# tmuird/VAEUNET

Measured on AMD Instinct MI355X. Metric: images/sec (whole node) at 3x512x512 bs=8/GPU; Dice parity vs CPU ref, higher is better.
Workload: dtype bf16; 1 GPU; UNet(3,2) train step (fwd+CombinedLoss+bwd+clip+AdamW), random-init weights; image=3x512x512, batch_per_gpu=8, global_batch=8, parallelism=dp1, execution=hipgraph-replay, wgrad_side_stream=False

## Files before the change

include/vaeunet.h:

```cpp
#ifndef VAEUNET_H
#define VAEUNET_H
#include <stdint.h>
#ifdef __cplusplus
extern "C" {
#endif

typedef struct VuGather {
  const void* src[3];
  int64_t stride[3];
  int32_t cend[3];
  int32_t nsrc;
  int32_t C;
  int32_t N, H, W;
  int32_t Hs, Ws;
  int32_t R, S;
  int32_t sy, sx, dy, dx, oy, ox;
} VuGather;

typedef struct VuGemmFwd {
  VuGather a;
  const void* b;
  int64_t ldb;
  int32_t ncol;
  int32_t out_mode;
// ... 216 lines not shown
                    int dtype, void* stream);
int vu_attn_gate_fwd(const float* q, const float* st, const void* x,
                     int64_t xs, int64_t P, int C, float* pmap, void* out,
                     int64_t os, int dtype, void* stream);
int vu_attn_gate_bwd(const void* dout, int64_t dos, const void* x, int64_t xs,
                     const float* pmap, int64_t P, int C, void* dx,
                     int64_t dxs, float* dqpre, int dtype, void* stream);
int64_t vu_attn_psi_bwd_workspace_bytes(int64_t P, int F);
int vu_attn_psi_bwd(const void* ug, const void* ux, int64_t P, int F,
                    const float* sg, const float* tg, const float* sx,
                    const float* tx, const float* wpsi, const float* dq,
                    void* ds, float* dwpsi, float* dbpsi, int accumulate,
                    float* workspace, int dtype, void* stream);
int64_t vu_attn_psi_bwd_blocks(int64_t P);
int vu_attn_psi_bwd_bnb_ok(int F);
int vu_attn_psi_bwd_bnb(const void* ug, const void* ux, int64_t P, int F,
                        const float* sg, const float* tg, const float* sx,
                        const float* tx, const float* wpsi, const float* dq,
                        void* ds, float* dwpsi, float* dbpsi, int accumulate,
                        float* workspace, const float* mean_g, const float* invstd_g,
                        const float* mean_x, const float* invstd_x, float* bnb_g,
                        float* bnb_x, int dtype, void* stream);

int64_t vu_attn_tail_bwd_tile(int F, int C);
int vu_attn_tail_bwd_ok(int64_t P, int F, int C, int64_t ldg, int64_t ldx, int64_t dos,
                        int64_t dgs, int64_t dg_coff, int64_t dxs, int dtype);
int vu_attn_tail_bwd(const void* ug, const void* ux, const float* dq, int64_t P, int F, int C,
                     const float* sg, const float* tg, const float* sx, const float* tx,
                     const float* wpsi, const float* mean_g, const float* coef_g,
                     const float* mean_x, const float* coef_x, const void* wdg, int64_t ldg,
                     const void* wdx, int64_t ldx, const void* dout, int64_t dos,
                     const float* pmap, void* dg, int64_t dgs, int64_t dg_coff, int dg_acc,
                     void* dx, int64_t dxs, void* dug, void* dux, int dtype, void* stream);

int vu_pointwise_fwd(const void* x, int64_t xs, int64_t P, int C, int J,
                     const float* w, const float* b, float* y, int64_t ys,
                     int dtype, void* stream);
int64_t vu_pointwise_bwd_workspace_bytes(int64_t P, int C, int J);
int vu_pointwise_bwd(const void* x, int64_t xs, const float* dy, int64_t dys,
                     int64_t P, int C, int J, const float* w, void* dx,
                     int64_t dxs, float* dw, float* db, int accumulate,
                     float* workspace, int dtype, void* stream);
int vu_pointwise_bn_fwd(const void* x, int64_t xs, int64_t P, int C, int J,
                        const float* bn_scale, const float* bn_shift, const float* w,
                        const float* b, float* y, int64_t ys, int dtype, void* stream);
int64_t vu_pointwise_bn_bwd_blocks(int64_t P);
int vu_pointwise_bn_bwd(const void* x, int64_t xs, const float* bn_coef, int64_t coef_stride,
                        const float* dy, int64_t dys, int64_t P, int C, int J, const float* w,
                        void* dx, int64_t dxs, float* dw, float* db, int accumulate,
                        float* workspace, float* bnb, int dtype, void* stream);

int64_t vu_loss_workspace_bytes(void);
int vu_bce_dice_fwd2(const float* logits, const float* target, int64_t n,
                     double* sums, float smooth, float w_bce, float w_dice,
                     float* loss, float* parts, double* workspace,
                     void* stream);
int vu_bce_dice_fwd(const float* logits, const float* target, int64_t n,
                    double* sums, double* workspace, void* stream);
int vu_bce_dice_bwd(const float* logits, const float* target, int64_t n,
                    const double* sums, float smooth, float w_bce,
                    float w_dice, const float* gscale, float* grad,
                    void* stream);
int vu_kl_free_bits2(const float* mu, const float* logvar, int B, int L,
                     float free_bits, const float* gscale, float* value,
                     float* gmu, float* glogvar, void* stream);
int vu_kl_free_bits(const float* mu, const float* logvar, int B, int L,
// ... 188 lines not shown
```

vaeunet_amd/_lib.py:

```python
import ctypes as C
import os

import torch

_HERE = os.path.dirname(os.path.abspath(__file__))
LIB_PATH = os.path.join(_HERE, "libvaeunet_hip.so")
if os.environ.get("VU_LIB_PATH"):
    LIB_PATH = os.environ["VU_LIB_PATH"]

F32, BF16 = 0, 1

_p = C.c_void_p
_i = C.c_int
_l = C.c_int64
_f = C.c_float


class VuGather(C.Structure):
    _fields_ = [("src", _p * 3), ("stride", _l * 3), ("cend", C.c_int32 * 3),
                ("nsrc", C.c_int32), ("C", C.c_int32),
                ("N", C.c_int32), ("H", C.c_int32), ("W", C.c_int32),
                ("Hs", C.c_int32), ("Ws", C.c_int32), ("R", C.c_int32), ("S", C.c_int32),
                ("sy", C.c_int32), ("sx", C.c_int32), ("dy", C.c_int32), ("dx", C.c_int32),
                ("oy", C.c_int32), ("ox", C.c_int32)]
# ... 102 lines not shown
    "vu_bn_bwd_reduce": (_i, [_p, _l, _p, _l, _l, _i, _p, _p, _p, _p, _p, _i, _i, _p, _p, _i,
                              _p, _p, _i, _p]),
    "vu_bn_bwd_apply": (_i, [_p, _l, _p, _l, _l, _i, _p, _p, _p, _p, _i, _p, _l, _i, _p]),
    "vu_bn_bwd_apply2_ok": (_i, [_i, _l, _l, _l, _l, _l]),
    "vu_bn_bwd_apply2": (_i, [_p, _l, _p, _l, _p, _l, _l, _i, _p, _p, _p, _p, _p, _l, _p, _l, _i, _p]),
    "vu_reduce_workspace_bytes": (_l, [_l, _i]),
    "vu_chan_sum": (_i, [_p, _l, _i, _i, _i, _i, _i, _i, _i, _i, _p, _i, _p, _i, _p]),
    "vu_copy": (_i, [_p, _l, _i, _p, _l, _i, _l, _i, _i, _p]),
    "vu_zero": (_i, [_p, _l, _l, _i, _i, _p]),
    "vu_gpu_delay": (_i, [_i, _p]),
    "vu_zero_insert2": (_i, [_p, _l, _i, _i, _i, _i, _p, _l, _i, _i, _i, _p]),
    "vu_input_pack": (_i, [_p, _l, _l, _l, _l, _i, _i, _i, _i, _i, _p, _i, _p]),
    "vu_maxpool2_fwd": (_i, [_p, _l, _i, _i, _i, _i, _p, _l, _i, _p]),
    "vu_maxpool2_bwd": (_i, [_p, _l, _p, _l, _i, _i, _i, _i, _p, _l, _p, _l, _i, _p]),
    "vu_bn_apply_maxpool2": (_i, [_p, _l, _p, _l, _p, _l, _i, _i, _i, _i, _p, _p, _i, _i, _p]),
    "vu_upsample_fwd": (_i, [_p, _l, _i, _i, _i, _i, _p, _l, _i, _i, _i, _i, _i, _i, _i, _p]),
    "vu_upsample_bwd": (_i, [_p, _l, _i, _i, _i, _i, _p, _l, _i, _i, _i, _i, _i, _i, _i, _i,
                             _p]),
    "vu_attn_tile_rows": (_l, []),
    "vu_attn_psi_fwd": (_i, [_p, _p, _l, _i, _p, _p, _p, _p, _p, _p, _p, _p, _p, _l, _i, _p]),
    "vu_attn_gate_fwd": (_i, [_p, _p, _p, _l, _l, _i, _p, _p, _l, _i, _p]),
    "vu_attn_gate_bwd": (_i, [_p, _l, _p, _l, _p, _l, _i, _p, _l, _p, _i, _p]),
    "vu_attn_psi_bwd_workspace_bytes": (_l, [_l, _i]),
    "vu_attn_psi_bwd_blocks": (_l, [_l]),
    "vu_attn_psi_bwd_bnb_ok": (_i, [_i]),
    "vu_attn_psi_bwd_bnb": (_i, [_p, _p, _l, _i, _p, _p, _p, _p, _p, _p, _p, _p, _p, _i, _p, _p, _p, _p, _p, _p, _p,
                                 _i, _p]),
    "vu_attn_psi_bwd": (_i, [_p, _p, _l, _i, _p, _p, _p, _p, _p, _p, _p, _p, _p, _i, _p, _i,
                             _p]),
    "vu_attn_tail_bwd_tile": (_l, [_i, _i]),
    "vu_attn_tail_bwd_ok": (_i, [_l, _i, _i, _l, _l, _l, _l, _l, _l, _i]),
    "vu_attn_tail_bwd": (_i, [_p, _p, _p, _l, _i, _i, _p, _p, _p, _p, _p, _p, _p, _p, _p, _p, _l, _p, _l, _p, _l,
                              _p, _p, _l, _l, _i, _p, _l, _p, _p, _i, _p]),
    "vu_pointwise_fwd": (_i, [_p, _l, _l, _i, _i, _p, _p, _p, _l, _i, _p]),
    "vu_pointwise_bwd_workspace_bytes": (_l, [_l, _i, _i]),
    "vu_pointwise_bn_fwd": (_i, [_p, _l, _l, _i, _i, _p, _p, _p, _p, _p, _l, _i, _p]),
    "vu_pointwise_bn_bwd_blocks": (_l, [_l]),
    "vu_pointwise_bn_bwd": (_i, [_p, _l, _p, _l, _p, _l, _l, _i, _i, _p, _p, _l, _p, _p, _i, _p, _p, _i, _p]),
    "vu_pointwise_bwd": (_i, [_p, _l, _p, _l, _l, _i, _i, _p, _p, _l, _p, _p, _i, _p, _i, _p]),
    "vu_loss_workspace_bytes": (_l, []),
    "vu_bce_dice_fwd2": (_i, [_p, _p, _l, _p, _f, _f, _f, _p, _p, _p, _p]),
    "vu_bce_dice_bwd": (_i, [_p, _p, _l, _p, _f, _f, _f, _p, _p, _p]),
    "vu_kl_free_bits2": (_i, [_p, _p, _i, _i, _f, _p, _p, _p, _p, _p]),
    "vu_sumsq": (_i, [_p, _l, _p, _p, _p]),
    "vu_dice_score": (_i, [_p, _p, _l, _f, _p, _p, _p, _p]),
    "vu_seg_counts_workspace_bytes": (_l, [_l]),
    "vu_seg_counts": (_i, [_p, _i, C.POINTER(_l), _i, _i, _p, _i, C.POINTER(_l), _i, _i, _i, _i, _i, _i, _p, _i, _p,
                           _p, _p]),
    "vu_seg_metrics": (_i, [_p, _i, _i, C.c_double, _p, _p, _i, _p, _p]),
    "vu_mt_chunk_elems": (_l, []),
    "vu_mt_grad_norm": (_i, [_p, _i, _l, _f, _p, _p, _p, _p]),
    "vu_mt_scale_grads": (_i, [_p, _i, _l, _p, _p]),
    "vu_mt_adamw": (_i, [_p, _i, _l, _f, _f, _f, _f, _f, _p, _p]),
    "vu_mt_adamw_dev": (_i, [_p, _i, _l, C.c_double, C.c_double, C.c_double, C.c_double, C.c_double, _p, _i,
                             _p]),
    "vu_mt_adamw_dev_scaled": (_i, [_p, _i, _l, C.c_double, C.c_double, C.c_double, C.c_double, C.c_double, _p,
                                    _i, _p, _p]),
    "vu_maxpool3s2_fwd": (_i, [_p, _l, _i, _i, _i, _i, _p, _l, _p, _i, _p]),
    "vu_maxpool3s2_bwd": (_i, [_p, _l, _p, _i, _i, _i, _i, _p, _l, _i, _i, _p]),
    "vu_bn_add_relu": (_i, [_p, _l, _p, _p, _p, _l, _p, _p, _l, _i, _p, _l, _i, _p]),
    "vu_relu_mask": (_i, [_p, _l, _p, _l, _l, _i, _p, _l, _i, _p]),
    "vu_sample_sum": (_i, [_p, _l, _i, _i, _i, _f, _p, _i, _p, _i, _p]),
    "vu_sample_sum_workspace_bytes": (_l, [_i, _i]),
    "vu_sample_broadcast": (_i, [_p, _i, _i, _i, _f, _p, _l, _i, _i, _p]),
    "vu_linear_small_fwd": (_i, [_p, _i, _i, _p, _p, _i, _p, _p]),
    "vu_linear_small_bwd": (_i, [_p, _i, _i, _p, _i, _p, _p, _i, _p, _p, _i, _p]),
# ... 67 lines not shown
```

vaeunet_amd/csrc/attention_tail.hip:

```cpp
#include <type_traits>

#include "host.h"
#include "attn_pre.h"

namespace {

VU_DEV uint32_t pack2(float a, float b) { return (uint32_t)f2bf(a) | ((uint32_t)f2bf(b) << 16); }

enum { Q_SG, Q_TG, Q_SX, Q_TX, Q_WP, Q_MG, Q_AG, Q_BG, Q_EG, Q_MX, Q_AX, Q_BX, Q_EX, NQ };

struct AttnTail {
  const bf16_t *ug, *ux;
  const float *dq, *pmap;
  const float* coef[NQ];
  const bf16_t *wg, *wx;
  int64_t ldg, ldx;
  const bf16_t* dout;
  int64_t dos;
  bf16_t* dg;
  int64_t dgs;
  int dg_acc;
  bf16_t* dx;
  int64_t dxs;
  bf16_t *dug, *dux;
  int64_t P;
};

template <int KS, int NJ, int NF, int NW>
__global__ __launch_bounds__(64 * NW, NW == 4 ? 2 : 1) void attn_tail_kernel(AttnTail p) {
  constexpr int K = 32 * KS, N = 16 * NJ, PX = 16 * NF, NT = 64 * NW;
  constexpr int GS = 4;
  static_assert(NJ % GS == 0, "whole 64-column groups");
  __shared__ __attribute__((aligned(16))) char wsm[2][N * K * 2];
  __shared__ __attribute__((aligned(16))) float csm[NQ][K];

  const int ntiles = (int)(p.P / PX);
  const int lane = threadIdx.x & 63;
  const int wid = __builtin_amdgcn_readfirstlane(threadIdx.x >> 6);
  const int gq = lane >> 4, r16 = lane & 15;

  auto wrow = [&](int j, int r) { return (j / GS) * 16 * GS + 4 * GS * (r >> 2) + 4 * (j % GS) + (r & 3); };
  {
    constexpr int PIECES = NJ * KS * 64;
#pragma unroll
    for (int img = 0; img < 2; ++img) {
      const bf16_t* bmat = img ? p.wx : p.wg;
      const int64_t ld = img ? p.ldx : p.ldg;
      for (int e = threadIdx.x; e < PIECES; e += NT) {
        const int l = e & 63, jk = e >> 6, j = jk / KS, ks = jk - j * KS;
        *reinterpret_cast<u32x4*>(wsm[img] + e * 16) =
            *reinterpret_cast<const u32x4*>(bmat + (int64_t)wrow(j, l & 15) * ld + 32 * ks + 8 * (l >> 4));
      }
    }
#pragma unroll
    for (int q = 0; q < NQ; ++q)
      for (int c = threadIdx.x; c < K; c += NT) csm[q][c] = p.coef[q][c];
    __syncthreads();
  }

  const int tstride = gridDim.x * NW;
  auto tile_px = [&](int t) {
    asm volatile("" : "+s"(t));
    return (int64_t)t * PX;
  };
  auto opq = [](uint32_t v) {
    asm volatile("" : "+v"(v));
    return v;
  };
  const uint32_t lk0 = (uint32_t)(r16 * K + 8 * gq);
  auto load = [&](int t, u32x4 (&a)[NF][KS], u32x4 (&b)[NF][KS], float (&g)[NF], float (&pv)[NF]) {
    const int64_t pb = tile_px(t);
    const uint32_t lk = opq(lk0), lr = opq((uint32_t)r16);
    const bf16_t *ugb = p.ug + pb * K + lk, *uxb = p.ux + pb * K + lk;
    const float *dqb = p.dq + pb + lr, *pmb = p.pmap + pb + lr;
#pragma unroll
    for (int f = 0; f < NF; ++f) {
      g[f] = dqb[16 * f];
      pv[f] = pmb[16 * f];
#pragma unroll
      for (int ks = 0; ks < KS; ++ks) {
        a[f][ks] = *reinterpret_cast<const u32x4*>(ugb + 16 * f * K + 32 * ks);
        b[f][ks] = *reinterpret_cast<const u32x4*>(uxb + 16 * f * K + 32 * ks);
      }
    }
  };
  u32x4 na[NF][KS], nb[NF][KS];
  float ng[NF], npv[NF];
  int tile = blockIdx.x * NW + wid;
  if (tile < ntiles) load(tile, na, nb, ng, npv);
  for (; tile < ntiles; tile += tstride) {
    const int64_t pb = tile_px(tile);
    int lo = 0;
    asm volatile("" : "+v"(lo));
    auto coef8 = [&](int q, int ks, float (&d)[8]) {
      const char* s = reinterpret_cast<const char*>(&csm[q][32 * ks + 8 * gq]) + lo;
      const f32x4 u = *reinterpret_cast<const f32x4*>(s), v = *reinterpret_cast<const f32x4*>(s + 16);
#pragma unroll
      for (int k = 0; k < 4; ++k) { d[k] = u[k]; d[4 + k] = v[k]; }
    };
    u32x4 ag[NF][KS], ax[NF][KS];
    float pv[NF];
#pragma unroll
    for (int f = 0; f < NF; ++f) pv[f] = npv[f];
#pragma unroll
    for (int ks = 0; ks < KS; ++ks) {
      Vec8<bf16_t> va[NF], vb[NF];
      float dsv[NF][8];
      {
        float wsg[8], wtg[8], wsx[8], wtx[8], wp[8];
        coef8(Q_SG, ks, wsg); coef8(Q_TG, ks, wtg); coef8(Q_SX, ks, wsx); coef8(Q_TX, ks, wtx); coef8(Q_WP, ks, wp);
#pragma unroll
        for (int f = 0; f < NF; ++f) {
          va[f].v = na[f][ks];
          vb[f].v = nb[f][ks];
#pragma unroll
          for (int k = 0; k < 8; ++k) {
            float s = attn_pre(va[f].get(k), wsg[k], wtg[k], vb[f].get(k), wsx[k], wtx[k]);
            bool on = s > 0.f;
            float gw = rnd<bf16_t>(ng[f] * wp[k]);
            asm volatile("" : "+v"(gw));
            dsv[f][k] = on ? gw : 0.f;
          }
        }
        __builtin_amdgcn_sched_barrier(0);
      }
#pragma unroll
      for (int side = 0; side < 2; ++side) {
        float mu[8], a[8], b[8], e[8];
        coef8(side ? Q_MX : Q_MG, ks, mu); coef8(side ? Q_AX : Q_AG, ks, a);
        coef8(side ? Q_BX : Q_BG, ks, b); coef8(side ? Q_EX : Q_EG, ks, e);
#pragma unroll
        for (int f = 0; f < NF; ++f) {
          const Vec8<bf16_t>& vx = side ? vb[f] : va[f];
          Vec8<bf16_t> o;
          o.zero();
#pragma unroll
          for (int k = 0; k < 8; ++k) {
            const float dz = dsv[f][k];
            o.set(k, fmaf(a[k], dz, b[k] * (vx.get(k) - mu[k])) + e[k]);
          }
          asm volatile("" : "+v"(o.v));
          (side ? ax : ag)[f][ks] = o.v;
        }
        __builtin_amdgcn_sched_barrier(0);
      }
    }
    if (tile + tstride < ntiles) load(tile + tstride, na, nb, ng, npv);
    {
      const uint32_t lk = opq(lk0);
      bf16_t *dugb = p.dug + pb * K + lk, *duxb = p.dux + pb * K + lk;
#pragma unroll
      for (int f = 0; f < NF; ++f)
#pragma unroll
        for (int ks = 0; ks < KS; ++ks) {
          *reinterpret_cast<u32x4*>(dugb + 16 * f * K + 32 * ks) = ag[f][ks];
          *reinterpret_cast<u32x4*>(duxb + 16 * f * K + 32 * ks) = ax[f][ks];
        }
    }

    auto add_old = [&](u32x4& v, const u32x4 o) {
#pragma unroll
      for (int w = 0; w < 4; ++w)
        v[w] = pack2(__uint_as_float(o[w] << 16) + __uint_as_float(v[w] << 16),
                     __uint_as_float(o[w] & 0xffff0000u) + __uint_as_float(v[w] & 0xffff0000u));
    };
    auto gemm = [&](const char* wimg, const u32x4 (&pf)[NF][KS], bf16_t* out, int64_t os, auto old_tag) {
      constexpr int OLD = decltype(old_tag)::value;
      f32x4 acc[NF][NJ];
#pragma unroll
      for (int f = 0; f < NF; ++f)
#pragma unroll
        for (int j = 0; j < NJ; ++j) acc[f][j] = f32x4{0, 0, 0, 0};
#pragma unroll
      for (int ks = 0; ks < KS; ++ks)
#pragma unroll
        for (int j = 0; j < NJ; ++j) {
          const u32x4 wf = *reinterpret_cast<const u32x4*>(wimg + lo + ((j * KS + ks) * 64 + lane) * 16);
#pragma unroll
          for (int f = 0; f < NF; ++f)
            acc[f][j] = __builtin_amdgcn_mfma_f32_16x16x32_bf16(__builtin_bit_cast(bf16x8, wf),
                                                                __builtin_bit_cast(bf16x8, pf[f][ks]), acc[f][j], 0, 0, 0);
          if constexpr (KS * NJ >= 64)
            if ((j & 7) == 7) __builtin_amdgcn_sched_barrier(0);
        }
#pragma unroll
      for (int f = 0; f < NF; ++f) {
        const uint32_t row = (uint32_t)(16 * f + r16);
        bf16_t* outp = out + pb * os + opq(row * (uint32_t)os + 8 * gq);
        const bf16_t* dop = p.dout + pb * p.dos + opq(row * (uint32_t)p.dos + 8 * gq);
// ... 22 lines not shown
#pragma unroll
            for (int gi = 0; gi < GC; ++gi)
#pragma unroll
              for (int h = 0; h < 2; ++h) {
                const int col = (g0 + gi) * 64 + 32 * h;
                if constexpr (OLD == 1) o[gi][h] = *reinterpret_cast<const u32x4*>(outp + col);
                else o[gi][h] = *reinterpret_cast<const u32x4*>(dop + col);
              }
#pragma unroll
            for (int gi = 0; gi < GC; ++gi)
#pragma unroll
              for (int h = 0; h < 2; ++h) {
                if constexpr (OLD == 2) {
#pragma unroll
                  for (int w = 0; w < 4; ++w)
                    o[gi][h][w] = pack2(__uint_as_float(o[gi][h][w] << 16) * pv[f],
                                        __uint_as_float(o[gi][h][w] & 0xffff0000u) * pv[f]);
                }
                add_old(c[gi][h], o[gi][h]);
              }
          }
#pragma unroll
          for (int gi = 0; gi < GC; ++gi)
#pragma unroll
            for (int h = 0; h < 2; ++h)
              *reinterpret_cast<u32x4*>(outp + (g0 + gi) * 64 + 32 * h) = c[gi][h];
        }
      }
    };
    if (p.dg_acc) gemm(wsm[0], ag, p.dg, p.dgs, std::integral_constant<int, 1>{});
    else gemm(wsm[0], ag, p.dg, p.dgs, std::integral_constant<int, 0>{});
    gemm(wsm[1], ax, p.dx, p.dxs, std::integral_constant<int, 2>{});
  }
}

constexpr int nf_of(int ks, int nj) {
  return (16 / nj < 4 ? 16 / nj : 4) < (4 / ks) ? (16 / nj < 4 ? 16 / nj : 4) : 4 / ks;
}
constexpr int nw_of(int ks, int nj) { return 2 * (16 * nj) * (32 * ks) * 2 > 72 * 1024 ? 8 : 4; }

template <int KS, int NJ>
int launch_nj(const AttnTail& p, hipStream_t st) {
  constexpr int NF = nf_of(KS, NJ), NW = nw_of(KS, NJ);
  const int64_t tiles = p.P / (16 * NF);
  int64_t nblk = (tiles + NW - 1) / NW;
  const int64_t cap = (NW == 4 ? 2 : 1) * (int64_t)cu_count();
  if (nblk > cap) nblk = cap;
  if (nblk == 0) return 0;
  hipLaunchKernelGGL((attn_tail_kernel<KS, NJ, NF, NW>), dim3((unsigned)nblk), dim3(64 * NW), 0, st, p);
  return (int)hipGetLastError();
}

template <int KS>
int launch_ks(const AttnTail& p, int C, hipStream_t st) {
  switch (C / 16) {
    case 4: return launch_nj<KS, 4>(p, st);
    case 8: return launch_nj<KS, 8>(p, st);
    case 16: return launch_nj<KS, 16>(p, st);
    default: return (int)hipErrorInvalidValue;
  }
}

}

extern "C" int64_t vu_attn_tail_bwd_tile(int F, int C) {
  if ((F != 32 && F != 64 && F != 128) || (C != 64 && C != 128 && C != 256)) return 0;
  return 16 * nf_of(F / 32, C / 16);
}

extern "C" int vu_attn_tail_bwd_ok(int64_t P, int F, int C, int64_t ldg, int64_t ldx, int64_t dos, int64_t dgs,
                                   int64_t dg_coff, int64_t dxs, int dtype) {
  if (dtype != VU_BF16) return 0;
  const int64_t px = vu_attn_tail_bwd_tile(F, C);
  if (px == 0) return 0;
  if (ldg % 8 != 0 || ldg < F || ldx % 8 != 0 || ldx < F) return 0;
  if (dos % 8 != 0 || dos < C || dgs % 8 != 0 || dg_coff % 8 != 0 || dg_coff < 0 || dgs < dg_coff + C || dxs % 8 != 0 ||
      dxs < C)
    return 0;
  if (dos >= (1 << 20) || dgs >= (1 << 20) || dxs >= (1 << 20)) return 0;
  if (P <= 0 || P % px != 0 || P >= ((int64_t)1 << 31)) return 0;
  return 1;
}

extern "C" int vu_attn_tail_bwd(const void* ug, const void* ux, const float* dq, int64_t P, int F, int C,
                                const float* sg, const float* tg, const float* sx, const float* tx,
                                const float* wpsi, const float* mean_g, const float* coef_g, const float* mean_x,
                                const float* coef_x, const void* wdg, int64_t ldg, const void* wdx, int64_t ldx,
                                const void* dout, int64_t dos, const float* pmap, void* dg, int64_t dgs,
                                int64_t dg_coff, int dg_acc, void* dx, int64_t dxs, void* dug, void* dux, int dtype,
                                void* stream) {
  if (!vu_attn_tail_bwd_ok(P, F, C, ldg, ldx, dos, dgs, dg_coff, dxs, dtype)) return (int)hipErrorInvalidValue;
  if (!ug || !ux || !dq || !sg || !tg || !sx || !tx || !wpsi || !mean_g || !coef_g || !mean_x || !coef_x || !wdg ||
      !wdx || !dout || !pmap || !dg || !dx || !dug || !dux)
    return (int)hipErrorInvalidValue;
  AttnTail p;
  p.ug = (const bf16_t*)ug; p.ux = (const bf16_t*)ux; p.dq = dq; p.pmap = pmap;
  p.coef[Q_SG] = sg; p.coef[Q_TG] = tg; p.coef[Q_SX] = sx; p.coef[Q_TX] = tx; p.coef[Q_WP] = wpsi;
  p.coef[Q_MG] = mean_g; p.coef[Q_AG] = coef_g; p.coef[Q_BG] = coef_g + F; p.coef[Q_EG] = coef_g + 2 * F;
  p.coef[Q_MX] = mean_x; p.coef[Q_AX] = coef_x; p.coef[Q_BX] = coef_x + F; p.coef[Q_EX] = coef_x + 2 * F;
  p.wg = (const bf16_t*)wdg; p.wx = (const bf16_t*)wdx; p.ldg = ldg; p.ldx = ldx;
  p.dout = (const bf16_t*)dout; p.dos = dos;
  p.dg = (bf16_t*)dg + dg_coff; p.dgs = dgs; p.dg_acc = dg_acc;
  p.dx = (bf16_t*)dx; p.dxs = dxs;
  p.dug = (bf16_t*)dug; p.dux = (bf16_t*)dux;
  p.P = P;
  hipStream_t st = (hipStream_t)stream;
  switch (F) {
    case 32: return launch_ks<1>(p, C, st);
    case 64: return launch_ks<2>(p, C, st);
    case 128: return launch_ks<4>(p, C, st);
    default: return (int)hipErrorInvalidValue;
  }
}
```

vaeunet_amd/engine.py:

```python
import warnings

import torch

from . import kernels as K
from ._lib import BF16, F32


OVERLAP_WGRAD = False

FUSE_BN_BWD_REDUCE = True


class SideStream:

    _per_device = {}

    def __init__(self, device):
        self.stream = torch.cuda.Stream(device=device)
        self.keep = []
        self.pending = False

    @classmethod
    def get(cls, device):
        key = torch.device(device).index
# ... 441 lines not shown


def double_conv_bwd(M, seq, saved, da2, need_dsrc, cvalid=None, da2_part=None):
    conv1, bn1, _, conv2, bn2, _ = seq
    srcs, a1, s1, s2 = saved
    da1, part = conv_bn_relu_bwd(M, [a1], conv2, bn2, s2, da2, True, feeds=(s1, bn1), da_part=da2_part)
    return conv_bn_relu_bwd(M, srcs, conv1, bn1, s1, da1, need_dsrc, cvalid, da_part=part)


def down_fwd(M, mod, x, pend=None, defer=False):
    seq = mod.maxpool_conv[1].double_conv
    if x is None:
        y, coef = pend
        N, C_, H, W = y.shape
        x = M.act(N, C_, H, W)
        xp = M.act(N, C_, H // 2, W // 2)
        K.bn_apply_maxpool(y, x, xp, coef, True, M.d)
    else:
        xp = K.maxpool_fwd(x, M.d)
    out, sdc = double_conv_fwd(M, seq, [xp], defer=defer)
    return x, out, (x, sdc)


def down_bwd(M, mod, saved, dout, add=None):
    x, sdc = saved
    seq = mod.maxpool_conv[1].double_conv
    dxp = double_conv_bwd(M, seq, sdc, dout, True)
    return PoolGrad(dxp, add, x)


FUSE_ATTN_BN_REDUCE = True
FUSE_ATTN_TAIL = True
ATTN_TAIL_MIN_TILES_PER_CU = 8


def _attn_tail_ok(M, P, F, g, x, dout, dg_out, wdg, wdx, dx):
    if not FUSE_ATTN_TAIL or M.d != BF16 or dg_out is None or g.shape[1] != x.shape[1]:
        return False
    C_ = x.shape[1]
    dst, coff = dg_out
    if not K.query("vu_attn_tail_bwd_ok", P, F, C_, wdg.shape[-1], wdx.shape[-1], K.pstride(dout),
                   K.pstride(dst), coff, K.pstride(dx), M.d):
        return False
    cus = torch.cuda.get_device_properties(x.device).multi_processor_count
    return P // K.query("vu_attn_tail_bwd_tile", F, C_) >= ATTN_TAIL_MIN_TILES_PER_CU * cus


def attention_fwd(M, att, g, x):
    N, _, H, W = x.shape
    P = N * H * W
    wg, bng = att.W_g[0], att.W_g[1]
    wx, bnx = att.W_x[0], att.W_x[1]
    wp, bnp = att.psi[0], att.psi[1]
    F = wg.out_channels
    ug = M.act(N, F, H, W)
    stg = K.gemm_fwd(K.gather1x1([g]), w1x1_fwd(wg.weight, M.d), F, ug, M.d, bias=wg.bias,
                     stats=bng.training)
    ux = M.act(N, F, H, W)
    stx = K.gemm_fwd(K.gather1x1([x]), w1x1_fwd(wx.weight, M.d), F, ux, M.d, bias=wx.bias,
                     stats=bnx.training)
    cg = bn_coef(bng, stg, F)
    cx = bn_coef(bnx, stx, F)
    tile = K.query("vu_attn_tile_rows")
    tiles = (P + tile - 1) // tile
    q = torch.empty((N, 1, H, W), dtype=torch.float32, device=x.device)
    psum = torch.empty(tiles, dtype=torch.float32, device=x.device)
# ... 23 lines not shown
    wg, bng = att.W_g[0], att.W_g[1]
    wx, bnx = att.W_x[0], att.W_x[1]
    wp, bnp = att.psi[0], att.psi[1]
    F = wg.out_channels
    dx = torch.empty_like(x)
    dbnq = torch.empty((N, 1, H, W), dtype=torch.float32, device=x.device)
    bnb = FUSE_ATTN_BN_REDUCE and K.query("vu_attn_psi_bwd_bnb_ok", F)
    tail = bool(bnb) and _attn_tail_ok(M, P, F, g, x, dout, dg_out, w1x1_dgrad(wg.weight, M.d),
                                       w1x1_dgrad(wx.weight, M.d), dx)
    K.call("vu_attn_gate_bwd", K.ptr(dout), K.pstride(dout), K.ptr(x), K.pstride(x), K.ptr(pmap),
           P, x.shape[1], None if tail else K.ptr(dx), K.pstride(dx), K.ptr(dbnq), M.d, K.stream())
    gw, accw = grad_sink(bnp.weight)
    gb, _ = grad_sink(bnp.bias)
    dq = torch.empty_like(q)
    K.bn_backward(dbnq, q, cq, bnp.weight, False, gw, gb, accw, dq, F32, train=bnp.training)
    ds = None if tail else M.act(N, F, H, W)
    gwp, accp = grad_sink(wp.weight)
    gbp, _ = grad_sink(wp.bias)
    ws = K.workspace_f32(K.query("vu_attn_psi_bwd_workspace_bytes", P, F), x.device)
    pg = px = None
    if bnb:
        nb = K.query("vu_attn_psi_bwd_blocks", P)
        bg = torch.empty((nb, 2, F), dtype=torch.float32, device=x.device)
        bx = torch.empty_like(bg)
        K.call("vu_attn_psi_bwd_bnb", K.ptr(ug), K.ptr(ux), P, F, K.ptr(cg[0]), K.ptr(cg[1]),
               K.ptr(cx[0]), K.ptr(cx[1]), K.ptr(wp.weight), K.ptr(dq), None if tail else K.ptr(ds),
               K.ptr(gwp), K.ptr(gbp), 1 if accp else 0, K.ptr(ws), K.ptr(cg[2]), K.ptr(cg[3]), K.ptr(cx[2]),
               K.ptr(cx[3]), K.ptr(bg), K.ptr(bx), M.d, K.stream())
        pg, px = K.BnbPart(bg, nb, ug), K.BnbPart(bx, nb, ux)
    else:
        K.call("vu_attn_psi_bwd", K.ptr(ug), K.ptr(ux), P, F, K.ptr(cg[0]), K.ptr(cg[1]),
               K.ptr(cx[0]), K.ptr(cx[1]), K.ptr(wp.weight), K.ptr(dq), K.ptr(ds), K.ptr(gwp),
               K.ptr(gbp), 1 if accp else 0, K.ptr(ws), M.d, K.stream())
    if tail:
        ks = []
        for u_, c_, bn_, part in ((ug, cg, bng, pg), (ux, cx, bnx, px)):
            gw_, gb_, acc_ = bn_grad_sinks(bn_)
            ks.append(K.bn_backward_finish(part, u_, c_, bn_.weight, gw_, gb_, acc_, train=bn_.training))
        dug, dux = torch.empty_like(ug), torch.empty_like(ux)
        wdg, wdx = w1x1_dgrad(wg.weight, M.d), w1x1_dgrad(wx.weight, M.d)
        dst, coff = dg_out

        def run_tail():
            K.call("vu_attn_tail_bwd", K.ptr(ug), K.ptr(ux), K.ptr(dq), P, F, x.shape[1], K.ptr(cg[0]),
                   K.ptr(cg[1]), K.ptr(cx[0]), K.ptr(cx[1]), K.ptr(wp.weight), K.ptr(cg[2]), K.ptr(ks[0]),
                   K.ptr(cx[2]), K.ptr(ks[1]), K.ptr(wdg), wdg.shape[-1], K.ptr(wdx), wdx.shape[-1],
                   K.ptr(dout), K.pstride(dout), K.ptr(pmap), K.ptr(dst), K.pstride(dst), coff,
                   1 if dg_acc else 0, K.ptr(dx), K.pstride(dx), K.ptr(dug), K.ptr(dux), M.d, K.stream())
        if K.AUDIT is None:
            run_tail()
        else:
            dx.copy_(dout.float() * pmap)
            K.audited_gemm(K.gather1x1([dug]), wdg, g.shape[1], dst, M.d, coff, dg_acc,
                           lambda: K.audited_gemm(K.gather1x1([dux]), wdx, x.shape[1], dx, M.d, 0, True, run_tail))
    elif pg is not None:
        dug, dux = bn_bwd_pair(ds, (ug, cg, bng, pg), (ux, cx, bnx, px), M)
    else:
        dug = bn_bwd(ds, ug, cg, bng, False, M)
        dux = bn_bwd(ds, ux, cx, bnx, False, M)

    def wgs():
        wgrad1x1(dug, [g], wg.weight, M)
        bias_grad(dug, wg.bias, M, bn=bng)
        wgrad1x1(dux, [x], wx.weight, M)
        bias_grad(dux, wx.bias, M, bn=bnx)
        M.notify([wg.weight, wg.bias, wx.weight, wx.bias, wp.weight, wp.bias, bng.weight, bng.bias,
                  bnx.weight, bnx.bias, bnp.weight, bnp.bias])
    M.side(wgs, dug, dux, g, x)
    if tail:
        return dx
    if dg_out is not None:
        dst, coff = dg_out
        K.gemm_fwd(K.gather1x1([dug]), w1x1_dgrad(wg.weight, M.d), g.shape[1], dst, M.d,
                   out_coff=coff, accumulate=dg_acc)
# ... 126 lines not shown
```

Before: 550.2 images/sec.

## Fuse 1x1 conv weight-gradient GEMMs into attention tail backward kernel

Adds a WG variant of the attention-tail backward kernel that computes the W_g and W_x 1x1 weight gradients in-kernel. It stages the bf16 dug/dux tiles and the g/x input tiles in LDS and runs transposed-read MFMA accumulation, then writes per-block partial slabs that a side-stream slab reduce sums. This removes the round trip of dug/dux through global memory and the separate weight-gradient GEMMs for the F=32, C=64 case. It costs extra LDS and registers, which may reduce occupancy, and halves the pixels per wave (NF capped at 2).

```diff
diff --git a/include/vaeunet.h b/include/vaeunet.h
--- a/include/vaeunet.h
+++ b/include/vaeunet.h
@@ -272,6 +272,20 @@
                      const void* wdx, int64_t ldx, const void* dout, int64_t dos,
                      const float* pmap, void* dg, int64_t dgs, int64_t dg_coff, int dg_acc,
                      void* dx, int64_t dxs, void* dug, void* dux, int dtype, void* stream);
+int vu_attn_tail_bwd_wg_ok(int64_t P, int F, int C, int64_t ldg, int64_t ldx, int64_t dos,
+                           int64_t dgs, int64_t dg_coff, int64_t dxs, int64_t gs, int64_t xs,
+                           int dtype);
+int64_t vu_attn_tail_bwd_wg_slabs(int64_t P, int F, int C);
+int64_t vu_attn_tail_bwd_wg_workspace_bytes(int64_t P, int F, int C);
+int vu_attn_tail_bwd_wg(const void* ug, const void* ux, const float* dq, int64_t P, int F, int C,
+                        const float* sg, const float* tg, const float* sx, const float* tx,
+                        const float* wpsi, const float* mean_g, const float* coef_g,
+                        const float* mean_x, const float* coef_x, const void* wdg, int64_t ldg,
+                        const void* wdx, int64_t ldx, const void* dout, int64_t dos,
+                        const float* pmap, void* dg, int64_t dgs, int64_t dg_coff, int dg_acc,
+                        void* dx, int64_t dxs, void* dug, void* dux, const void* g, int64_t gs,
+                        const void* x, int64_t xs, float* ws, int64_t ws_bytes, int dtype,
+                        void* stream);
 
 int vu_pointwise_fwd(const void* x, int64_t xs, int64_t P, int C, int J,
                      const float* w, const float* b, float* y, int64_t ys,
diff --git a/vaeunet_amd/_lib.py b/vaeunet_amd/_lib.py
--- a/vaeunet_amd/_lib.py
+++ b/vaeunet_amd/_lib.py
@@ -158,6 +158,11 @@
     "vu_attn_tail_bwd_ok": (_i, [_l, _i, _i, _l, _l, _l, _l, _l, _l, _i]),
     "vu_attn_tail_bwd": (_i, [_p, _p, _p, _l, _i, _i, _p, _p, _p, _p, _p, _p, _p, _p, _p, _p, _l, _p, _l, _p, _l,
                               _p, _p, _l, _l, _i, _p, _l, _p, _p, _i, _p]),
+    "vu_attn_tail_bwd_wg_ok": (_i, [_l, _i, _i, _l, _l, _l, _l, _l, _l, _l, _l, _i]),
+    "vu_attn_tail_bwd_wg_slabs": (_l, [_l, _i, _i]),
+    "vu_attn_tail_bwd_wg_workspace_bytes": (_l, [_l, _i, _i]),
+    "vu_attn_tail_bwd_wg": (_i, [_p, _p, _p, _l, _i, _i, _p, _p, _p, _p, _p, _p, _p, _p, _p, _p, _l, _p, _l, _p, _l,
+                                 _p, _p, _l, _l, _i, _p, _l, _p, _p, _p, _l, _p, _l, _p, _l, _i, _p]),
     "vu_pointwise_fwd": (_i, [_p, _l, _l, _i, _i, _p, _p, _p, _l, _i, _p]),
     "vu_pointwise_bwd_workspace_bytes": (_l, [_l, _i, _i]),
     "vu_pointwise_bn_fwd": (_i, [_p, _l, _l, _i, _i, _p, _p, _p, _p, _p, _l, _i, _p]),
diff --git a/vaeunet_amd/csrc/attention_tail.hip b/vaeunet_amd/csrc/attention_tail.hip
--- a/vaeunet_amd/csrc/attention_tail.hip
+++ b/vaeunet_amd/csrc/attention_tail.hip
@@ -4,6 +4,24 @@
 #include "attn_pre.h"
 
 namespace {
+
+typedef __attribute__((address_space(3))) void lds_void;
+
+template <int RB> VU_DEV int fsw(int m) {
+  return RB >= 256 ? ((m & 3) | ((m >> 1) & 4))
+                   : RB == 128 ? (((m >> 1) & 1) | ((m >> 2) & 2)) : ((m >> 3) & 1);
+}
+template <int RB> VU_DEV int tr_off(int m, int col) {
+  return m * RB + (((col >> 4) ^ fsw<RB>(m)) << 5) + ((col & 15) << 1);
+}
+VU_DEV u32x2 tr_read(const char* p) {
+  u32x2 r;
+  const uint32_t a = (uint32_t)(uintptr_t)(const lds_void*)p;
+  asm volatile("ds_read_b64_tr_b16 %0, %1" : "=v"(r) : "v"(a) : "memory");
+  return r;
+}
+VU_DEV void lgkm_drain() { asm volatile("s_waitcnt lgkmcnt(0)" ::: "memory"); }
+VU_DEV void tie(u32x2& v) { asm volatile("" : "+v"(v)); }
 
 VU_DEV uint32_t pack2(float a, float b) { return (uint32_t)f2bf(a) | ((uint32_t)f2bf(b) << 16); }
 
@@ -24,15 +42,25 @@
   int64_t dxs;
   bf16_t *dug, *dux;
   int64_t P;
+  const bf16_t *g, *x;
+  int64_t gs, xs;
+  float* slab;
 };
 
-template <int KS, int NJ, int NF, int NW>
+template <int KS, int NJ, int NF, int NW, bool WG>
 __global__ __launch_bounds__(64 * NW, NW == 4 ? 2 : 1) void attn_tail_kernel(AttnTail p) {
   constexpr int K = 32 * KS, N = 16 * NJ, PX = 16 * NF, NT = 64 * NW;
   constexpr int GS = 4;
   static_assert(NJ % GS == 0, "whole 64-column groups");
   __shared__ __attribute__((aligned(16))) char wsm[2][N * K * 2];
   __shared__ __attribute__((aligned(16))) float csm[NQ][K];
+  constexpr int RBA = 2 * K, RBB = 2 * N, STG = PX * (RBA + RBB);
+  constexpr int TI = 2 * KS, TJ = NJ;
+  constexpr int CH = N / 8, RPI = 64 / CH;
+  constexpr int NLD = WG ? PX / RPI : 1;
+  static_assert(!WG || PX % 32 == 0, "whole k-steps of 32 pixels");
+  constexpr int STGS = !WG ? 16 : STG > K * N * 4 ? NW * STG : NW * K * N * 4;
+  __shared__ __attribute__((aligned(16))) char stg[STGS];
 
   const int ntiles = (int)(p.P / PX);
   const int lane = threadIdx.x & 63;
@@ -84,10 +112,34 @@
       }
     }
   };
+  auto load_gx = [&](int t, u32x4 (&gt)[NLD], u32x4 (&xt)[NLD]) {
+    const int64_t pb = tile_px(t);
+    const uint32_t row = (uint32_t)(lane / CH), col = (uint32_t)(8 * (lane % CH));
+    const bf16_t* gb = p.g + pb * p.gs + opq(row * (uint32_t)p.gs + col);
+    const bf16_t* xb = p.x + pb * p.xs + opq(row * (uint32_t)p.xs + col);
+#pragma unroll
+    for (int i = 0; i < NLD; ++i) {
+      gt[i] = *reinterpret_cast<const u32x4*>(gb + (uint32_t)(RPI * i) * (uint32_t)p.gs);
+      xt[i] = *reinterpret_cast<const u32x4*>(xb + (uint32_t)(RPI * i) * (uint32_t)p.xs);
+    }
+  };
   u32x4 na[NF][KS], nb[NF][KS];
   float ng[NF], npv[NF];
+  u32x4 ngt[NLD], nxt[NLD];
+  f32x4 wacc[2][TI][TJ];
+  if constexpr (WG) {
+#pragma unroll
+    for (int sd = 0; sd < 2; ++sd)
+#pragma unroll
+      for (int a = 0; a < TI; ++a)
+#pragma unroll
+        for (int b = 0; b < TJ; ++b) wacc[sd][a][b] = f32x4{0, 0, 0, 0};
+  }
   int tile = blockIdx.x * NW + wid;
-  if (tile < ntiles) load(tile, na, nb, ng, npv);
+  if (tile < ntiles) {
+    load(tile, na, nb, ng, npv);
+    if constexpr (WG) load_gx(tile, ngt, nxt);
+  }
   for (; tile < ntiles; tile += tstride) {
     const int64_t pb = tile_px(tile);
     int lo = 0;
@@ -145,16 +197,71 @@
         __builtin_amdgcn_sched_barrier(0);
       }
     }
-    if (tile + tstride < ntiles) load(tile + tstride, na, nb, ng, npv);
+    if constexpr (WG) {
+      char* sa = stg + wid * STG;
+      char* sb = sa + PX * RBA;
+      const int ln = (int)opq((uint32_t)lane);
+      const int gq = ln >> 4, r16 = ln & 15, qd = r16 >> 2, pp = r16 & 3;
+#pragma unroll
+      for (int sd = 0; sd < 2; ++sd) {
+#pragma unroll
+        for (int f = 0; f < NF; ++f)
+#pragma unroll
+          for (int ks = 0; ks < KS; ++ks)
+            *reinterpret_cast<u32x4*>(sa + tr_off<RBA>(16 * f + r16, 32 * ks + 8 * gq)) = (sd ? ax : ag)[f][ks];
+#pragma unroll
+        for (int i = 0; i < NLD; ++i)
+          *reinterpret_cast<u32x4*>(sb + tr_off<RBB>(RPI * i + ln / CH, 8 * (ln % CH))) = (sd ? nxt : ngt)[i];
+        lgkm_drain();
+#pragma unroll
+        for (int kk = 0; kk < PX / 32; ++kk) {
+          const int m = 32 * kk + 8 * gq + qd;
+          u32x2 al[TI], ah[TI], bl[TJ], bh[TJ];
+#pragma unroll
+          for (int a = 0; a < TI; ++a) {
+            al[a] = tr_read(sa + tr_off<RBA>(m, 16 * a + 4 * pp));
+            ah[a] = tr_read(sa + tr_off<RBA>(m + 4, 16 * a + 4 * pp));
+          }
+#pragma unroll
+          for (int b = 0; b < TJ; ++b) {
+            bl[b] = tr_read(sb + tr_off<RBB>(m, 16 * b + 4 * pp));
+            bh[b] = tr_read(sb + tr_off<RBB>(m + 4, 16 * b + 4 * pp));
+          }
+          lgkm_drain();
+          u32x4 af[TI], bf[TJ];
+#pragma unroll
+          for (int a = 0; a < TI; ++a) {
+            tie(al[a]); tie(ah[a]);
+            af[a] = u32x4{al[a][0], al[a][1], ah[a][0], ah[a][1]};
+          }
+#pragma unroll
+          for (int b = 0; b < TJ; ++b) {
+            tie(bl[b]); tie(bh[b]);
+            bf[b] = u32x4{bl[b][0], bl[b][1], bh[b][0], bh[b][1]};
+          }
+#pragma unroll
+          for (int a = 0; a < TI; ++a)
+#pragma unroll
+            for (int b = 0; b < TJ; ++b)
+              wacc[sd][a][b] = __builtin_amdgcn_mfma_f32_16x16x32_bf16(
+                  __builtin_bit_cast(bf16x8, af[a]), __builtin_bit_cast(bf16x8, bf[b]), wacc[sd][a][b], 0, 0, 0);
+        }
+      }
+    }
+    if (tile + tstride < ntiles) {
+      load(tile + tstride, na, nb, ng, npv);
+      if constexpr (WG) load_gx(tile + tstride, ngt, nxt);
+    }
     {
       const uint32_t lk = opq(lk0);
       bf16_t *dugb = p.dug + pb * K + lk, *duxb = p.dux + pb * K + lk;
+      const bool st_g = !WG || p.dug != nullptr, st_x = !WG || p.dux != nullptr;
 #pragma unroll
       for (int f = 0; f < NF; ++f)
 #pragma unroll
         for (int ks = 0; ks < KS; ++ks) {
-          *reinterpret_cast<u32x4*>(dugb + 16 * f * K + 32 * ks) = ag[f][ks];
-          *reinterpret_cast<u32x4*>(duxb + 16 * f * K + 32 * ks) = ax[f][ks];
+          if (st_g) *reinterpret_cast<u32x4*>(dugb + 16 * f * K + 32 * ks) = ag[f][ks];
+          if (st_x) *reinterpret_cast<u32x4*>(duxb + 16 * f * K + 32 * ks) = ax[f][ks];
         }
     }
 
@@ -243,6 +350,28 @@
     else gemm(wsm[0], ag, p.dg, p.dgs, std::integral_constant<int, 0>{});
     gemm(wsm[1], ax, p.dx, p.dxs, std::integral_constant<int, 2>{});
   }
+  if constexpr (WG) {
+    float* red = reinterpret_cast<float*>(stg);
+#pragma unroll
+    for (int sd = 0; sd < 2; ++sd) {
+      __syncthreads();
+#pragma unroll
+      for (int a = 0; a < TI; ++a)
+#pragma unroll
+        for (int b = 0; b < TJ; ++b)
+#pragma unroll
+          for (int r = 0; r < 4; ++r)
+            red[(wid * K + 16 * a + 4 * gq + r) * N + 16 * b + r16] = wacc[sd][a][b][r];
+      __syncthreads();
+      float* out = p.slab + ((int64_t)sd * gridDim.x + blockIdx.x) * (K * N);
+      for (int e = threadIdx.x; e < K * N / 4; e += NT) {
+        f32x4 s = *reinterpret_cast<const f32x4*>(red + 4 * e);
+#pragma unroll
+        for (int w = 1; w < NW; ++w) s += *reinterpret_cast<const f32x4*>(red + w * K * N + 4 * e);
+        *reinterpret_cast<f32x4*>(out + 4 * e) = s;
+      }
+    }
+  }
 }
 
 constexpr int nf_of(int ks, int nj) {
@@ -250,15 +379,20 @@
 }
 constexpr int nw_of(int ks, int nj) { return 2 * (16 * nj) * (32 * ks) * 2 > 72 * 1024 ? 8 : 4; }
 
-template <int KS, int NJ>
+constexpr int nf_wg(int ks, int nj) { return nf_of(ks, nj) < 2 ? nf_of(ks, nj) : 2; }
+
+int64_t grid_of(int64_t P, int nf, int nw) {
+  const int64_t tiles = P / (16 * nf);
+  const int64_t nblk = (tiles + nw - 1) / nw, cap = (nw == 4 ? 2 : 1) * (int64_t)cu_count();
+  return nblk > cap ? cap : nblk;
+}
+
+template <int KS, int NJ, bool WG = false>
 int launch_nj(const AttnTail& p, hipStream_t st) {
-  constexpr int NF = nf_of(KS, NJ), NW = nw_of(KS, NJ);
-  const int64_t tiles = p.P / (16 * NF);
-  int64_t nblk = (tiles + NW - 1) / NW;
-  const int64_t cap = (NW == 4 ? 2 : 1) * (int64_t)cu_count();
-  if (nblk > cap) nblk = cap;
+  constexpr int NF = WG ? nf_wg(KS, NJ) : nf_of(KS, NJ), NW = nw_of(KS, NJ);
+  const int64_t nblk = grid_of(p.P, NF, NW);
   if (nblk == 0) return 0;
-  hipLaunchKernelGGL((attn_tail_kernel<KS, NJ, NF, NW>), dim3((unsigned)nblk), dim3(64 * NW), 0, st, p);
+  hipLaunchKernelGGL((attn_tail_kernel<KS, NJ, NF, NW, WG>), dim3((unsigned)nblk), dim3(64 * NW), 0, st, p);
   return (int)hipGetLastError();
 }
 
@@ -293,16 +427,16 @@
   return 1;
 }
 
-extern "C" int vu_attn_tail_bwd(const void* ug, const void* ux, const float* dq, int64_t P, int F, int C,
-                                const float* sg, const float* tg, const float* sx, const float* tx,
-                                const float* wpsi, const float* mean_g, const float* coef_g, const float* mean_x,
-                                const float* coef_x, const void* wdg, int64_t ldg, const void* wdx, int64_t ldx,
-                                const void* dout, int64_t dos, const float* pmap, void* dg, int64_t dgs,
-                                int64_t dg_coff, int dg_acc, void* dx, int64_t dxs, void* dug, void* dux, int dtype,
-                                void* stream) {
-  if (!vu_attn_tail_bwd_ok(P, F, C, ldg, ldx, dos, dgs, dg_coff, dxs, dtype)) return (int)hipErrorInvalidValue;
+namespace {
+
+int tail_run(const void* ug, const void* ux, const float* dq, int64_t P, int F, int C, const float* sg,
+             const float* tg, const float* sx, const float* tx, const float* wpsi, const float* mean_g,
+             const float* coef_g, const float* mean_x, const float* coef_x, const void* wdg, int64_t ldg,
+             const void* wdx, int64_t ldx, const void* dout, int64_t dos, const float* pmap, void* dg, int64_t dgs,
+             int64_t dg_coff, int dg_acc, void* dx, int64_t dxs, void* dug, void* dux, const void* g, int64_t gs,
+             const void* x, int64_t xs, float* slab, bool wg, void* stream) {
   if (!ug || !ux || !dq || !sg || !tg || !sx || !tx || !wpsi || !mean_g || !coef_g || !mean_x || !coef_x || !wdg ||
-      !wdx || !dout || !pmap || !dg || !dx || !dug || !dux)
+      !wdx || !dout || !pmap || !dg || !dx)
     return (int)hipErrorInvalidValue;
   AttnTail p;
   p.ug = (const bf16_t*)ug; p.ux = (const bf16_t*)ux; p.dq = dq; p.pmap = pmap;
@@ -315,7 +449,9 @@
   p.dx = (bf16_t*)dx; p.dxs = dxs;
   p.dug = (bf16_t*)dug; p.dux = (bf16_t*)dux;
   p.P = P;
+  p.g = (const bf16_t*)g; p.x = (const bf16_t*)x; p.gs = gs; p.xs = xs; p.slab = slab;
   hipStream_t st = (hipStream_t)stream;
+  if (wg) return launch_nj<1, 4, true>(p, st);
   switch (F) {
     case 32: return launch_ks<1>(p, C, st);
     case 64: return launch_ks<2>(p, C, st);
@@ -323,3 +459,54 @@
     default: return (int)hipErrorInvalidValue;
   }
 }
+
+}
+
+extern "C" int vu_attn_tail_bwd(const void* ug, const void* ux, const float* dq, int64_t P, int F, int C,
+                                const float* sg, const float* tg, const float* sx, const float* tx,
+                                const float* wpsi, const float* mean_g, const float* coef_g, const float* mean_x,
+                                const float* coef_x, const void* wdg, int64_t ldg, const void* wdx, int64_t ldx,
+                                const void* dout, int64_t dos, const float* pmap, void* dg, int64_t dgs,
+                                int64_t dg_coff, int dg_acc, void* dx, int64_t dxs, void* dug, void* dux, int dtype,
+                                void* stream) {
+  if (!vu_attn_tail_bwd_ok(P, F, C, ldg, ldx, dos, dgs, dg_coff, dxs, dtype)) return (int)hipErrorInvalidValue;
+  if (!dug || !dux) return (int)hipErrorInvalidValue;
+  return tail_run(ug, ux, dq, P, F, C, sg, tg, sx, tx, wpsi, mean_g, coef_g, mean_x, coef_x, wdg, ldg, wdx, ldx, dout,
+                  dos, pmap, dg, dgs, dg_coff, dg_acc, dx, dxs, dug, dux, nullptr, 0, nullptr, 0, nullptr, false,
+                  stream);
+}
+
+extern "C" int vu_attn_tail_bwd_wg_ok(int64_t P, int F, int C, int64_t ldg, int64_t ldx, int64_t dos, int64_t dgs,
+                                      int64_t dg_coff, int64_t dxs, int64_t gs, int64_t xs, int dtype) {
+  if (!vu_attn_tail_bwd_ok(P, F, C, ldg, ldx, dos, dgs, dg_coff, dxs, dtype)) return 0;
+  if (F != 32 || C != 64) return 0;
+  if (gs % 8 != 0 || gs < C || xs % 8 != 0 || xs < C || gs >= (1 << 20) || xs >= (1 << 20)) return 0;
+  return 1;
+}
+
+extern "C" int64_t vu_attn_tail_bwd_wg_slabs(int64_t P, int F, int C) {
+  if (F != 32 || C != 64 || P <= 0 || P % vu_attn_tail_bwd_tile(F, C) != 0) return 0;
+  return grid_of(P, nf_wg(F / 32, C / 16), nw_of(F / 32, C / 16));
+}
+
+extern "C" int64_t vu_attn_tail_bwd_wg_workspace_bytes(int64_t P, int F, int C) {
+  return 2 * vu_attn_tail_bwd_wg_slabs(P, F, C) * F * C * (int64_t)sizeof(float);
+}
+
+extern "C" int vu_attn_tail_bwd_wg(const void* ug, const void* ux, const float* dq, int64_t P, int F, int C,
+                                   const float* sg, const float* tg, const float* sx, const float* tx,
+                                   const float* wpsi, const float* mean_g, const float* coef_g, const float* mean_x,
+                                   const float* coef_x, const void* wdg, int64_t ldg, const void* wdx, int64_t ldx,
+                                   const void* dout, int64_t dos, const float* pmap, void* dg, int64_t dgs,
+                                   int64_t dg_coff, int dg_acc, void* dx, int64_t dxs, void* dug, void* dux,
+                                   const void* g, int64_t gs, const void* x, int64_t xs, float* ws, int64_t ws_bytes,
+                                   int dtype, void* stream) {
+  if (!vu_attn_tail_bwd_wg_ok(P, F, C, ldg, ldx, dos, dgs, dg_coff, dxs, gs, xs, dtype))
+    return (int)hipErrorInvalidValue;
+  if (!g || !x || !ws || reinterpret_cast<uintptr_t>(g) % 16 != 0 || reinterpret_cast<uintptr_t>(x) % 16 != 0 ||
+      reinterpret_cast<uintptr_t>(ws) % 16 != 0 ||
+      ws_bytes < vu_attn_tail_bwd_wg_workspace_bytes(P, F, C))
+    return (int)hipErrorInvalidValue;
+  return tail_run(ug, ux, dq, P, F, C, sg, tg, sx, tx, wpsi, mean_g, coef_g, mean_x, coef_x, wdg, ldg, wdx, ldx, dout,
+                  dos, pmap, dg, dgs, dg_coff, dg_acc, dx, dxs, dug, dux, g, gs, x, xs, ws, true, stream);
+}
diff --git a/vaeunet_amd/engine.py b/vaeunet_amd/engine.py
--- a/vaeunet_amd/engine.py
+++ b/vaeunet_amd/engine.py
@@ -497,6 +497,8 @@
 FUSE_ATTN_BN_REDUCE = True
 FUSE_ATTN_TAIL = True
 ATTN_TAIL_MIN_TILES_PER_CU = 8
+FUSE_ATTN_TAIL_WGRAD = True
+ATTN_TAIL_WGRAD_MIN_TILES_PER_CU = 8
 
 
 def _attn_tail_ok(M, P, F, g, x, dout, dg_out, wdg, wdx, dx):
@@ -586,14 +588,46 @@
         K.call("vu_attn_psi_bwd", K.ptr(ug), K.ptr(ux), P, F, K.ptr(cg[0]), K.ptr(cg[1]),
                K.ptr(cx[0]), K.ptr(cx[1]), K.ptr(wp.weight), K.ptr(dq), K.ptr(ds), K.ptr(gwp),
                K.ptr(gbp), 1 if accp else 0, K.ptr(ws), M.d, K.stream())
+    wgf = False
     if tail:
         ks = []
         for u_, c_, bn_, part in ((ug, cg, bng, pg), (ux, cx, bnx, px)):
             gw_, gb_, acc_ = bn_grad_sinks(bn_)
             ks.append(K.bn_backward_finish(part, u_, c_, bn_.weight, gw_, gb_, acc_, train=bn_.training))
-        dug, dux = torch.empty_like(ug), torch.empty_like(ux)
         wdg, wdx = w1x1_dgrad(wg.weight, M.d), w1x1_dgrad(wx.weight, M.d)
         dst, coff = dg_out
+        wgf = (FUSE_ATTN_TAIL_WGRAD and K.AUDIT is None and bng.training and bnx.training
+               and wg.weight.requires_grad and wx.weight.requires_grad
+               and P // K.query("vu_attn_tail_bwd_tile", F, x.shape[1]) >= ATTN_TAIL_WGRAD_MIN_TILES_PER_CU
+               * torch.cuda.get_device_properties(x.device).multi_processor_count
+               and bool(K.query("vu_attn_tail_bwd_wg_ok", P, F, x.shape[1], wdg.shape[-1], wdx.shape[-1],
+                                K.pstride(dout), K.pstride(dst), coff, K.pstride(dx), K.pstride(g),
+                                K.pstride(x), M.d)))
+    if wgf:
+        C_ = x.shape[1]
+        nsl = K.query("vu_attn_tail_bwd_wg_slabs", P, F, C_)
+        nbytes = K.query("vu_attn_tail_bwd_wg_workspace_bytes", P, F, C_)
+        slabs = K.workspace_f32(nbytes, x.device)[:2 * nsl * F * C_].view(2, nsl, F, C_)
+        K.call("vu_attn_tail_bwd_wg", K.ptr(ug), K.ptr(ux), K.ptr(dq), P, F, C_, K.ptr(cg[0]),
+               K.ptr(cg[1]), K.ptr(cx[0]), K.ptr(cx[1]), K.ptr(wp.weight), K.ptr(cg[2]), K.ptr(ks[0]),
+               K.ptr(cx[2]), K.ptr(ks[1]), K.ptr(wdg), wdg.shape[-1], K.ptr(wdx), wdx.shape[-1],
+               K.ptr(dout), K.pstride(dout), K.ptr(pmap), K.ptr(dst), K.pstride(dst), coff,
+               1 if dg_acc else 0, K.ptr(dx), K.pstride(dx), None, None, K.ptr(g), K.pstride(g),
+               K.ptr(x), K.pstride(x), K.ptr(slabs), nbytes, M.d, K.stream())
+
+        def wgs_fused():
+            for side, (conv, bn_) in enumerate(((wg, bng), (wx, bnx))):
+                gr, acc = grad_sink(conv.weight)
+                s_i, s_tap, s_c = conv_layout(gr)
+                K.call("vu_slab_reduce", K.ptr(slabs[side]), nsl, F, C_, C_, C_, s_i, s_tap, s_c, K.ptr(gr),
+                       1 if acc else 0, K.stream())
+                bias_grad(None, conv.bias, M, bn=bn_)
+            M.notify([wg.weight, wg.bias, wx.weight, wx.bias, wp.weight, wp.bias, bng.weight, bng.bias,
+                      bnx.weight, bnx.bias, bnp.weight, bnp.bias])
+        M.side(wgs_fused, slabs)
+        return dx
+    if tail:
+        dug, dux = torch.empty_like(ug), torch.empty_like(ux)
 
         def run_tail():
             K.call("vu_attn_tail_bwd", K.ptr(ug), K.ptr(ux), K.ptr(dq), P, F, x.shape[1], K.ptr(cg[0]),
```

Result: no change. 554.1 images/sec, median of 6 (+0.7%).
